# david-m-rosen/Optimization

Hardware: AMD Instinct MI355X
Metric: TNT Steihaug-CG HVP+inner-product throughput (higher is better)
Workload: dtype f64

## Files before the change

### optimization_amd/csrc/context.hip

```cpp
#include "mi_internal.h"
#include <chrono>
#include <cstring>
#include <strings.h>
#include <unistd.h>

#include <dlfcn.h>

namespace mi {

static thread_local char g_err[1024] = "";

void set_error(const char *fmt, ...) {
  va_list ap;
  va_start(ap, fmt);
  vsnprintf(g_err, sizeof(g_err), fmt, ap);
  va_end(ap);
}

int hip_fail(hipError_t e, const char *what, const char *file, int line) {
  set_error("HIP error %d (%s) in %s at %s:%d", (int)e, hipGetErrorString(e), what, file, line);
  (void)hipGetLastError();
  if (e == hipErrorNoDevice || e == hipErrorInvalidDevice) return MI_ERR_NO_DEVICE;
  if (e == hipErrorOutOfMemory) return MI_ERR_OOM;
  return MI_ERR_HIP;
// ... 171 lines not shown
using namespace mi;

namespace {
struct OptionDesc {
  const char *name;
  int (*set)(mi_ctx *, long);
  bool integer = false;
};
#define OPT_BOOL(FN, FIELD) \
  int FN(mi_ctx *c, long v) { c->FIELD = v != 0; return MI_OK; }
OPT_BOOL(opt_force_slot_path, force_slot_path)
OPT_BOOL(opt_force_lockstep, force_lockstep)
OPT_BOOL(opt_no_dirgram, no_dirgram)
OPT_BOOL(opt_dirgram_direct, dirgram_direct)
OPT_BOOL(opt_force_uniform_grid, cfg.force_uniform_grid)
OPT_BOOL(opt_no_fold, cfg.no_fold)
OPT_BOOL(opt_halo_push_late, cfg.halo_push_late)
OPT_BOOL(opt_no_packed, cfg.no_packed)
OPT_BOOL(opt_no_window, cfg.no_window)
OPT_BOOL(opt_no_win_bounds, cfg.no_win_bounds)
OPT_BOOL(opt_no_far_computed, cfg.no_far_computed)
OPT_BOOL(opt_words16, cfg.words16)
OPT_BOOL(opt_no_spmm_stream, cfg.no_spmm_stream)
OPT_BOOL(opt_no_spmm_win, cfg.no_spmm_win)
OPT_BOOL(opt_no_spmm_sweep, cfg.no_spmm_sweep)
OPT_BOOL(opt_no_zero_copy, cfg.no_zero_copy)
OPT_BOOL(opt_no_polled_sync, cfg.no_polled_sync)
OPT_BOOL(opt_no_update_mfma, cfg.no_update_mfma)
OPT_BOOL(opt_halo_rprime, cfg.halo_rprime)
OPT_BOOL(opt_no_gram_half, cfg.no_gram_half)
OPT_BOOL(opt_so3_no_quat, cfg.so3_no_quat)
OPT_BOOL(opt_so3_no_rquat, cfg.so3_no_rquat)
OPT_BOOL(opt_early_s, cfg.early_s)
OPT_BOOL(opt_no_update_pair, cfg.no_update_pair)
OPT_BOOL(opt_two_kernel_step, cfg.two_kernel_step)
OPT_BOOL(opt_warn_generic, warn_generic)
#undef OPT_BOOL
int opt_max_grid(mi_ctx *c, long v) {
  c->max_grid = (int)std::min<long>(kMaxGrid, std::max<long>(1, v));
  return MI_OK;
}
int opt_wide_quad(mi_ctx *c, long v) {
  c->cfg.wide_quad = v < 0 ? -1 : v != 0;
  return MI_OK;
}
int opt_wide_window(mi_ctx *c, long v) {
  c->cfg.wide_window = v < 0 ? -1 : v != 0;
  return MI_OK;
}
int opt_so3_sort_nbr(mi_ctx *c, long v) {
  c->cfg.so3_sort_nbr = (int)v;
  return MI_OK;
}
int opt_sweep_zsegs(mi_ctx *c, long v) {
  c->cfg.sweep_zsegs = (int)std::max<long>(0, std::min<long>(v, 1024));
  return MI_OK;
}
int opt_reanchor(mi_ctx *c, long v) {
  c->cfg.reanchor = (int)std::max<long>(0, std::min<long>(v, 1 << 20));
  return MI_OK;
}
int opt_ipc_timeout_ms(mi_ctx *c, long v) {
  c->cfg.ipc_timeout_ms = std::max<long>(0, v);
  return MI_OK;
}
const OptionDesc kOptions[] = {
    {"FORCE_SLOT_PATH", opt_force_slot_path}, {"FORCE_LOCKSTEP", opt_force_lockstep},
    {"NO_DIRGRAM", opt_no_dirgram}, {"DIRGRAM_DIRECT", opt_dirgram_direct}, {"MAX_GRID", opt_max_grid, true},
    {"FORCE_UNIFORM_GRID", opt_force_uniform_grid}, {"IPC_TIMEOUT_MS", opt_ipc_timeout_ms, true},
    {"NO_FOLD", opt_no_fold}, {"HALO_PUSH_LATE", opt_halo_push_late}, {"NO_PACKED", opt_no_packed},
    {"NO_WINDOW", opt_no_window}, {"NO_WIN_BOUNDS", opt_no_win_bounds}, {"NO_FAR_COMPUTED", opt_no_far_computed},
    {"WORDS16", opt_words16}, {"NO_SPMM_STREAM", opt_no_spmm_stream}, {"NO_SPMM_WIN", opt_no_spmm_win},
    {"NO_SPMM_SWEEP", opt_no_spmm_sweep}, {"SWEEP_ZSEGS", opt_sweep_zsegs, true},
    {"NO_ZERO_COPY", opt_no_zero_copy}, {"NO_POLLED_SYNC", opt_no_polled_sync}, {"WIDE_QUAD", opt_wide_quad, true}, {"WIDE_WINDOW", opt_wide_window, true},
    {"NO_UPDATE_MFMA", opt_no_update_mfma}, {"HALO_RPRIME", opt_halo_rprime}, {"NO_GRAM_HALF", opt_no_gram_half}, {"SO3_NO_QUAT", opt_so3_no_quat}, {"SO3_NO_RQUAT", opt_so3_no_rquat}, {"EARLY_S", opt_early_s}, {"NO_UPDATE_PAIR", opt_no_update_pair}, {"TWO_KERNEL_STEP", opt_two_kernel_step}, {"SO3_SORT_NBR", opt_so3_sort_nbr, true},
    {"WARN_GENERIC", opt_warn_generic}, {"REANCHOR", opt_reanchor, true},
};
bool option_value(const OptionDesc &o, const char *e, long *v) {
  char *end = nullptr;
  *v = strtol(e, &end, 0);
  if (end != e && *end == '\0') return true;
  if (o.integer) {
    fprintf(stderr, "[mi355opt] warning: MI355OPT_%s=\"%s\" is not an integer; ignored (the default stays)\n", o.name, e);
    return false;
  }
  *v = (!strcasecmp(e, "no") || !strcasecmp(e, "false") || !strcasecmp(e, "off")) ? 0 : 1;
  return true;
}
void config_from_env(mi_ctx *ctx) {
  for (const OptionDesc &o : kOptions) {
    char name[64];
    snprintf(name, sizeof(name), "MI355OPT_%s", o.name);
    long v = 0;
    if (const char *e = getenv(name))
      if (option_value(o, e, &v)) (void)o.set(ctx, v);
  }
  static bool warned = false;
  if (warned || !environ) return;
  warned = true;
  for (char **ep = environ; *ep; ++ep) {
    if (strncmp(*ep, "MI355OPT_", 9) != 0) continue;
    const char *nm = *ep + 9, *eq = strchr(nm, '=');
    const size_t len = eq ? (size_t)(eq - nm) : strlen(nm);
    bool known = false;
    for (const OptionDesc &o : kOptions) known |= strlen(o.name) == len && strncmp(o.name, nm, len) == 0;
    for (const char *h : {"LIB", "COMM", "BUILD_TAG", "EXTRA_CFLAGS", "NO_UNITY"})
      known |= strlen(h) == len && strncmp(h, nm, len) == 0;
    known |= len >= 6 && strncmp(nm, "BENCH_", 6) == 0;
// ... 297 lines not shown
```

### optimization_amd/csrc/mi_internal.h

```cpp
#pragma once

#include <hip/hip_runtime.h>

#include <cstdarg>
#include <cstdint>
#include <cstdio>
#include <cstring>
#include <map>
#include <string>
#include <set>
#include <vector>

#include "mi355opt.h"

namespace mi {

constexpr int kWave = 64;
constexpr int kBlock = 1024;
constexpr int kWaves = kBlock / kWave;
constexpr int kMaxP = 8;
constexpr int kMaxGrid = 512;
constexpr int kMaxRows = 1024;
constexpr int kMaxComps = 64;
constexpr int kNumXCD = 8;
// ... 8 lines not shown
    if (_e != hipSuccess) return ::mi::hip_fail(_e, #expr, __FILE__, __LINE__); \
  } while (0)

#define MI_TRY(expr)          \
  do {                        \
    int _s = (expr);          \
    if (_s != MI_OK) return _s; \
  } while (0)

#define MI_REQUIRE(cond, ...)              \
  do {                                     \
    if (!(cond)) {                         \
      ::mi::set_error(__VA_ARGS__);        \
      return MI_ERR_INVALID_ARGUMENT;      \
    }                                      \
  } while (0)

struct HostStatus {
  volatile uint64_t word;
  volatile uint32_t epoch;
};

struct CgState {
  double sk_M_pk, sk_M_2, pk_M_2;
  double target_rk_norm;
  double rv;
  double alpha, beta, kappa, sigma;
  double skplus1_M_2;
  double M_norm;
  unsigned long long k;
  unsigned long long launches;
  int mode;
  int exit_reason;
};
static_assert(sizeof(CgState) <= 128, "the CG state is meant to fit one 128-byte line");
struct CgConst {
  double Delta, Delta_2, epsilon;
  unsigned long long max_iterations;
  unsigned long long rag0, rag_per;
};
enum CgMode { CG_RUN = 0, CG_KERNEL_PENDING = 1, CG_APPLY_SIGMA = 2, CG_DONE = 3 };

struct Config {
  bool force_uniform_grid = false;
  long ipc_timeout_ms = 0;
  bool no_fold = false;
  bool halo_push_late = false;
  bool no_packed = false;
  bool no_window = false;
  bool no_win_bounds = false;
  bool no_far_computed = false;
  bool words16 = false;
  bool no_spmm_stream = false;
  bool no_spmm_sweep = true;
  int sweep_zsegs = 0;
  bool no_spmm_win = false;
  bool no_zero_copy = false;
  int wide_quad = -1;
  int wide_window = -1;
  bool no_polled_sync = false;
  bool two_kernel_step = false;
  int reanchor = 25;
  bool no_update_pair = false;
  bool no_gram_half = false;
  bool no_update_mfma = false;
  bool halo_rprime = false;
  bool early_s = false;
  bool so3_no_rquat = false;
  bool so3_no_quat = false;
  int so3_sort_nbr = 0;
};

struct KTimer {
  bool enabled = false;
  std::vector<std::pair<hipEvent_t, hipEvent_t>> pending;
  size_t launches = 0;
  double total_ms = 0;
};

}

struct mi_ctx {
  int device = -1;
  hipStream_t stream = nullptr;
  char device_name[128] = {0};
  int num_cu = 256;
  bool uniform_grid = false;
  int max_grid = 512;
  std::multimap<size_t, void *> pool_free;
  std::map<void *, size_t> pool_all;
  size_t pool_bytes = 0;
  void *control_slab = nullptr;
  double *partials = nullptr;
  double *partials_b = nullptr;
  double *partials2 = nullptr;
  double *partials_user = nullptr;
  double *scalars = nullptr;
  double *host_scalars = nullptr;
  mi::CgState *cg = nullptr;
  mi::CgState *cg1 = nullptr;
// ... 366 lines not shown
```

### optimization_amd/csrc/stpcg.hip

```cpp
#include "comm_ipc.h"
#include "mi_internal.h"
#include "stiefel_core.h"

#include <cmath>
#include <type_traits>

using namespace mi;

namespace {

enum { PRE_NONE = 0, PRE_DIAG = 1, PRE_BLOCK3 = 2, PRE_EXTERNAL = 3 };

__device__ __forceinline__ void publish(HostStatus *hs, unsigned long long launches, int done) {
  __hip_atomic_store(&hs->word, (uint64_t)(launches << 1) | (uint64_t)(done ? 1 : 0), __ATOMIC_RELAXED,
                     __HIP_MEMORY_SCOPE_SYSTEM);
}

#define CG_FIELDS(X)                                                                               \
  X(sk_M_pk) X(sk_M_2) X(pk_M_2) X(target_rk_norm) X(rv) X(alpha) X(beta)                          \
  X(kappa) X(sigma) X(skplus1_M_2) X(M_norm) X(k) X(launches) X(mode) X(exit_reason)
__device__ __forceinline__ CgState load_state(const CgState *__restrict__ src) {
  CgState s;
#define X(f) s.f = src->f;
  CG_FIELDS(X)
// ... 258 lines not shown
    s.exit_reason = MI_STPCG_EXIT_RESIDUAL;
    s.M_norm = sqrt(0.0);
  }
  store_state(st, s);
  publish(hs, 0, s.mode == CG_DONE);
}

struct DirGramArgs {
  const double *X, *Y, *S;
  double *gpartials;
  double *gdir;
  int ns;
};

#ifdef MI_FOLD_STAMPS
}
extern "C" __attribute__((visibility("default"))) int mi_debug_fold_stamp_buffer(void *dev_ptr) {
  return (int)hipMemcpyToSymbol(HIP_SYMBOL(mi::g_fold_stamps), &dev_ptr, sizeof(dev_ptr));
}
namespace {
#endif

template <int SP>
struct DirGramLds {
  static constexpr int value = (SymIdx<SP>::NS * kWaves > kWaves + 1) ? SymIdx<SP>::NS * kWaves : kWaves + 1;
};
template <>
struct DirGramLds<0> {
  static constexpr int value = kWaves + 1;
};
static_assert(kWaves + 1 >= kIpcVals, "LDS of the folded exchange");

#define CG_KERNEL_ATTR
#define CG_UPDATE_NAME k_cg_update
#define CG_PUPDATE_NAME k_cg_pupdate
#include "stpcg_kernels.inc"
#undef CG_KERNEL_ATTR
#undef CG_UPDATE_NAME
#undef CG_PUPDATE_NAME
#define CG_KERNEL_ATTR __attribute__((amdgpu_num_sgpr(80), amdgpu_waves_per_eu(8, 8)))
#define CG_UPDATE_NAME k_cg_update_s80
#define CG_PUPDATE_NAME k_cg_pupdate_s80
#include "stpcg_kernels.inc"
#undef CG_KERNEL_ATTR
#undef CG_UPDATE_NAME
#undef CG_PUPDATE_NAME

template <class F>
__device__ __forceinline__ void reduce_rows_1x512(const double *__restrict__ partials, int count, double &out, double *lds,
                                                  F &&after_issue) {
  const int lane = threadIdx.x & 63, w = threadIdx.x >> 6;
  double t[8];
#pragma unroll
  for (int j = 0; j < 8; ++j) t[j] = 0.0;
  if (w == 0) {
#pragma unroll
    for (int j = 0; j < 8; ++j) {
      const int r = lane + 64 * j;
      if (r < count) t[j] = partials[r];
    }
  }
  after_issue();
  if (w == 0) {
    double v = 0;
#pragma unroll
    for (int j = 0; j < 8; ++j) v += t[j];
    v = wave_reduce_sum(v);
    if (lane == 0) lds[0] = v;
  }
  __syncthreads();
  out = lds[0];
  __syncthreads();
}

__global__ __launch_bounds__(kBlock) __attribute__((amdgpu_waves_per_eu(8, 8))) void k_cg_pupdate_early(
    size_t n, CgConst cc, const CgState *__restrict__ st_in, CgState *__restrict__ st_out,
    const double *__restrict__ partials_b, int nparts_b, const double *__restrict__ v, double *__restrict__ p,
    double *__restrict__ s, HostStatus *hs, double *__restrict__ trace, size_t trace_cap, DirGramArgs dg) {
  __shared__ double lds[kWaves + 1];
// ... 57 lines not shown
      trace[3 * trace_cap + k] = cs.rv;
    }
    publish(hs, cs.launches, cs.mode == CG_DONE);
    if (dg.gdir && mode_in == CG_RUN && cs.mode == CG_RUN) {
      for (int i = 0; i < dg.ns; ++i) dg.gdir[SLOT_GDIR_P + i] = -dg.gdir[i] + cs.beta * dg.gdir[SLOT_GDIR_P + i];
    }
  }
  if (mode_in == CG_KERNEL_PENDING) {
    const double sigma = cs.sigma;
    for (unsigned i = i0; i < n2; i += stride) {
      const double2 pv = reinterpret_cast<const double2 *>(p)[i];
      double2 sv = reinterpret_cast<double2 *>(s)[i];
      sv.x += sigma * pv.x; sv.y += sigma * pv.y;
      reinterpret_cast<double2 *>(s)[i] = sv;
    }
    if ((n & 1) && leader) s[n - 1] += sigma * p[n - 1];
  } else if (mode_in == CG_RUN) {
    const double alpha = cs.alpha, beta = cs.beta;
    const bool dir = cs.mode == CG_RUN;
    if (dir) {
#pragma unroll
      for (int j = 0; j < 3; ++j)
        if (Le[j] < n2) {
          double2 pv = pe[j];
          const double2 vv = ve[j];
          pv.x = -vv.x + beta * pv.x; pv.y = -vv.y + beta * pv.y;
          reinterpret_cast<double2 *>(p)[Le[j]] = pv;
        }
    }
    if ((n & 1) && leader) {
      s[n - 1] = s[n - 1] + alpha * p[n - 1];
      if (dir) p[n - 1] = -v[n - 1] + beta * p[n - 1];
    }
  }
}


template <int NS>
__global__ __launch_bounds__(kBlock) void k_cg_step2(size_t n, CgConst cc, const CgState *__restrict__ st_in,
                                                     CgState *__restrict__ st_out, const double *__restrict__ partials_a,
                                                     int nparts_a, const double *__restrict__ Hp, double *__restrict__ r,
                                                     double *__restrict__ p, double *__restrict__ s, HostStatus *hs,
                                                     double *__restrict__ trace, size_t trace_cap, DirGramArgs dg) {
  constexpr int KC = 3 + NS + 2;
  __shared__ double lds[3 * (kWaves + 1)];
  static_assert(KC <= kWaves, "one wave per component");
  CgState cs = load_state(st_in);
  const bool leader = blockIdx.x == 0 && threadIdx.x == 0;
  if (cs.mode == CG_DONE) {
    if (leader) store_state(st_out, cs);
    return;
  }
  const size_t n2 = n >> 1, stride = (size_t)gridDim.x * kBlock, i0 = (size_t)blockIdx.x * kBlock + threadIdx.x;
  double2 hv0 = make_double2(0, 0), rv0 = hv0, pv0 = hv0, sv0 = hv0;
  auto prefetch = [&] {
    if (i0 < n2) {
      hv0 = reinterpret_cast<const double2 *>(Hp)[i0];
      rv0 = reinterpret_cast<double2 *>(r)[i0];
      pv0 = reinterpret_cast<double2 *>(p)[i0];
      sv0 = reinterpret_cast<double2 *>(s)[i0];
    }
  };
  double d[KC];
  reduce_rows<KC>(partials_a, nparts_a, d, lds, prefetch);
  step_a(cs, cc, d[0], d[1], d[2]);
  const int mode_a = cs.mode;
// ... 316 lines not shown
  touch(s_out);
  ctx->fusion.fused_stpcg_solves++;
  MI_REQUIRE(!P || (P->ctx == ctx && P->n == g->n), "preconditioner dimension/context mismatch");
  MI_REQUIRE(!prm->constraint_At || (P && P->apply_project),
             "constraint_At needs a constraint preconditioner (mi_precon_create_constraint)");
  MI_REQUIRE(!(P && P->kind == 3 && ctx->world_size > 1),
             "the constraint preconditioner is single-rank: its reductions are not completed across ranks");
  MI_REQUIRE(prm->Delta > 0, "Trust-region radius (Delta) must be a positive real value");
  MI_REQUIRE(prm->kappa_fgr >= 0 && prm->kappa_fgr < 1,
             "Target fractional reduction of the gradient norm (kappa_fgr) must be a real value in "
             "the range [0,1)");
  MI_REQUIRE(prm->theta >= 0 && prm->theta <= 1,
             "Target superlinear convergence rate (theta) must be a real value in the range [0,1]");
  MI_REQUIRE(prm->epsilon > 0 && prm->epsilon < 1,
             "Relative norm tolerance for declaring a vector to lie in the kernel of H (epsilon) "
             "should be a small positive number in the range (0,1)");

  RangeScope range("mi_stpcg");
  comm_halo_fold_drop(ctx);
  const size_t n = g->n;
  const int pre = !P ? PRE_NONE : (P->kind == 1 ? PRE_DIAG : (P->kind == 2 ? PRE_BLOCK3 : PRE_EXTERNAL));
  MI_REQUIRE(pre != PRE_BLOCK3 || n % 3 == 0, "block-Jacobi preconditioner needs n divisible by 3");
  const bool sharded = slot_mode(ctx);
  const bool rows = rows_mode(ctx);
  const mi_dirgram *dgp = (!ctx->no_dirgram && H->dirgram && H->apply_dir) ? H->dirgram : nullptr;
  if (dgp && dgp->p > 4 && (pre != PRE_NONE || ctx->dirgram_direct)) dgp = nullptr;
  MI_REQUIRE(!dgp || (dgp->p >= 1 && dgp->p <= kMaxP && dgp->n * (size_t)dgp->p == g->n),
             "operator's direction-Gram description does not match the problem dimension");
  const int run_ahead = prm->run_ahead > 0 ? prm->run_ahead : 3;
  const bool lockstep = (ctx->comm != nullptr && ctx->world_size > 1) || ctx->force_lockstep;

  if (P && P->fail_word) MI_HIP(hipMemsetAsync(P->fail_word, 0, sizeof(double), ctx->stream));

  mi_vec *r = nullptr, *v = nullptr, *p = nullptr, *Hp = nullptr;
  MI_TRY(mi_vec_create(ctx, n, &r));
  MI_TRY(mi_vec_create(ctx, n, &p));
  MI_TRY(mi_vec_create(ctx, n, &Hp));
  if (pre != PRE_NONE) MI_TRY(mi_vec_create(ctx, n, &v));
  double *vd = (pre == PRE_NONE) ? r->d : v->d;
  const double *pred = P ? P->data : nullptr;

  size_t tcap = 0;
  if (trace && trace->cap) {
    if (ctx->trace_cap < trace->cap) {
      if (ctx->trace_dev) MI_HIP(hipFree(ctx->trace_dev));
      MI_HIP(hipMalloc((void **)&ctx->trace_dev, 4 * trace->cap * sizeof(double)));
      ctx->trace_cap = trace->cap;
    }
    tcap = ctx->trace_cap;
  }

  ctx->cg_deferred = false;
  ctx->cg_deferred_seq = 0;
  ctx->epoch++;
  ctx->status->word = 0;
  ctx->status->epoch = ctx->epoch;

  CgSetup cfg{prm->Delta, prm->kappa_fgr, prm->theta, prm->epsilon,
              (unsigned long long)prm->max_iterations};
  CgConst cc{prm->Delta, prm->Delta * prm->Delta, prm->epsilon, (unsigned long long)prm->max_iterations, 0ull, 0ull};
  hipStream_t st = ctx->stream;
  const int grid = (pre == PRE_BLOCK3) ? grid_for(ctx, n / 3, 2) : grid_for(ctx, n, 4);
  {
    const size_t n2 = n >> 1, step = (size_t)grid * kBlock;
    cc.rag0 = (n2 / step) * step;
    cc.rag_per = (n2 - cc.rag0 + (size_t)grid - 1) / (size_t)grid;
  }
  const bool recur = dgp && pre == PRE_NONE && !ctx->dirgram_direct;
  const int gns = dgp ? dgp->p * (dgp->p + 1) / 2 : 0;
  const DirGramArgs dga = dgp ? DirGramArgs{dgp->X, dgp->Y, dgp->S, ctx->partials2,
                                            recur ? ctx->scalars + SLOT_GDIR : nullptr, gns}
                              : DirGramArgs{nullptr, nullptr, nullptr, nullptr, nullptr, 0};
  const int sp = (dgp && !recur) ? dgp->p : 0;
  const int kc = recur ? dir_comps(dgp->p) : 3;
  double *slots_g = ctx->scalars + SLOT_GRAM;
  double *slots_a = ctx->scalars + SLOT_CG, *slots_b = ctx->scalars + SLOT_CG + 4;
  CgState *st0 = ctx->cg, *st1 = ctx->cg1;
  const bool folded = sharded && recur && kc <= kIpcVals && comm_fold_enabled(ctx) && !ctx->force_slot_path;
  bool rprime = false;
  if (recur && !folded && dgp->halo_A) {
    const int st_rp = comm_rprime_prepare(ctx, dgp->halo_A, &rprime);
    if (st_rp != MI_OK) {
      mi_vec_destroy(r);
      mi_vec_destroy(p);
      mi_vec_destroy(Hp);
      if (v) mi_vec_destroy(v);
      return st_rp;
    }
  }
  const bool init_fused = recur && n == dgp->n * (size_t)dgp->p;
  const bool gdir_in_scalar_init = recur && !sharded && !rows;
  const bool twok = ctx->cfg.two_kernel_step && recur && dgp->twok && dgp->p == 3 && !sharded && !rows && !lockstep &&
                    init_fused && gdir_in_scalar_init;
  CgState *st_final = st0;
  double *tr = tcap ? ctx->trace_dev : nullptr;
  int ret = MI_OK;
  ctx->cg_live = st0;

#define CG_CHECK(expr)   \
  do {                   \
    int _s = (expr);     \
    if (_s != MI_OK) {   \
      ret = _s;          \
      goto cleanup;      \
    }                    \
  } while (0)
#define LAUNCH_PRE(KERNEL, ...)                                                                   \
  switch (pre) {                                                                                  \
    case PRE_NONE: hipLaunchKernelGGL((KERNEL<PRE_NONE>), dim3(grid), dim3(kBlock), 0, st, __VA_ARGS__); break;     \
    case PRE_DIAG: hipLaunchKernelGGL((KERNEL<PRE_DIAG>), dim3(grid), dim3(kBlock), 0, st, __VA_ARGS__); break;     \
    case PRE_BLOCK3: hipLaunchKernelGGL((KERNEL<PRE_BLOCK3>), dim3(grid), dim3(kBlock), 0, st, __VA_ARGS__); break; \
    default: hipLaunchKernelGGL((KERNEL<PRE_EXTERNAL>), dim3(grid), dim3(kBlock), 0, st, __VA_ARGS__); break;       \
  }
#define LAUNCH_UPDATE(FS)                                                                              \
  switch (pre) {                                                                                       \
    case PRE_NONE: hipLaunchKernelGGL((k_cg_update<PRE_NONE, FS>), dim3(grid), dim3(kBlock), 0, st, UPD_ARGS, NoFold{}); break;     \
    case PRE_DIAG: hipLaunchKernelGGL((k_cg_update<PRE_DIAG, FS>), dim3(grid), dim3(kBlock), 0, st, UPD_ARGS, NoFold{}); break;     \
    case PRE_BLOCK3: hipLaunchKernelGGL((k_cg_update<PRE_BLOCK3, FS>), dim3(grid), dim3(kBlock), 0, st, UPD_ARGS, NoFold{}); break; \
    default: hipLaunchKernelGGL((k_cg_update<PRE_EXTERNAL, FS>), dim3(grid), dim3(kBlock), 0, st, UPD_ARGS, NoFold{}); break;       \
  }

  if (init_fused) {
    KScope ks(ctx, MI_K_CG_INIT);
    const size_t nrows = dgp->n;
#define INIT_DG(SPV)                                                                                       \
  hipLaunchKernelGGL(k_cg_init_dirgram<SPV>, dim3(grid), dim3(StBlk<SPV>::threads), 0, st, nrows, (const double *)g->d, \
                     r->d, p->d, s_out->d, ctx->partials_b, dga)
    switch (dgp->p) {
      case 1: INIT_DG(1); break;
      case 2: INIT_DG(2); break;
      case 3: INIT_DG(3); break;
      case 4: INIT_DG(4); break;
      case 5: INIT_DG(5); break;
      case 6: INIT_DG(6); break;
      case 7: INIT_DG(7); break;
      default: INIT_DG(8); break;
    }
#undef INIT_DG
  } else {
    KScope ks(ctx, MI_K_CG_INIT);
    LAUNCH_PRE(k_cg_init, n, (const double *)g->d, pred, r->d, vd, p->d, s_out->d, ctx->partials_b);
  }
  if (pre == PRE_EXTERNAL) {
    if (P->apply_project) CG_CHECK(P->apply_project(P, r, v, prm->constraint_At));
    else CG_CHECK(P->apply(P, r, v));
    hipLaunchKernelGGL(k_cg_dot_rv<true>, dim3(grid), dim3(kBlock), 0, st, n, (const CgState *)st0,
                       (const double *)r->d, (const double *)v->d, p->d, ctx->partials_b);
  }
  if (dgp) {
    const size_t nrows = dgp->n;
    if (!init_fused) {
      switch (dgp->p) {
// ... 70 lines not shown
            hipLaunchKernelGGL(k_cg_gdir_anchor, dim3(1), dim3(kBlock), 0, st, (const double *)ctx->partials2, grid, gns,
                               (const double *)slots_g, sharded ? 1 : 0, (const CgState *)st0,
                               dga.gdir + (which == 0 ? SLOT_GDIR_P : 0), (double *)nullptr);
          }
        }
      }

      int nparts = 0;
      if (twok) {
        CgState *cur = (k & 1) ? st1 : st0, *nxt = (k & 1) ? st0 : st1;
        ctx->cg_live = cur;
        ctx->twok_r = r->d;
        CG_CHECK(H->apply_dir(H, p, Hp, -2, &nparts));
        ctx->twok_r = nullptr;
        ++hvp;
        {
          KScope ks(ctx, MI_K_CG_UPDATE);
          hipLaunchKernelGGL(k_cg_step2<6>, dim3(grid), dim3(kBlock), 0, st, n, cc, (const CgState *)cur, nxt,
                             (const double *)ctx->partials, nparts, (const double *)Hp->d, r->d, p->d, s_out->d,
                             ctx->status_dev, tr, tcap, dga);
        }
        st_final = nxt;
        continue;
      }
      if (dgp) {
        CG_CHECK(H->apply_dir(H, p, Hp, recur ? -1 : grid, &nparts));
      } else if (H->apply_dots) {
        CG_CHECK(H->apply_dots(H, p, Hp, &nparts));
      } else {
        CG_CHECK(H->apply(H, p, Hp));
        CG_CHECK(launch_dot3_partials(ctx, n, p->d, Hp->d, &nparts));
      }
      ++hvp;
#define UPD_ARGS                                                                                      \
  n, cc, (const CgState *)st0, st1, (const double *)ctx->partials, nparts,                              \
      (const double *)(recur ? slots_g : slots_a), (const double *)p->d, (const double *)Hp->d, pred,  \
      s_out->d, r->d, vd, ctx->partials_b, dga
      if (recur) {
#define UPD_RECUR(KN, FS, FT, FV)                                                                                  \
  switch (kc) {                                                                                                    \
    case 4: hipLaunchKernelGGL((KN<PRE_NONE, FS, 4, FT>), dim3(grid), dim3(kBlock), 0, st, UPD_ARGS, FV); break;   \
    case 6: hipLaunchKernelGGL((KN<PRE_NONE, FS, 6, FT>), dim3(grid), dim3(kBlock), 0, st, UPD_ARGS, FV); break;   \
    case 9: hipLaunchKernelGGL((KN<PRE_NONE, FS, 9, FT>), dim3(grid), dim3(kBlock), 0, st, UPD_ARGS, FV); break;   \
    default: hipLaunchKernelGGL((k_cg_update_s80<PRE_NONE, FS, 16, FT>), dim3(grid), dim3(kBlock), 0, st, UPD_ARGS, FV); break; \
  }
#define UPD_WIDE(FS)                                                                                                        \
  switch (kc) {                                                                                                             \
    case 18: hipLaunchKernelGGL((k_cg_update<PRE_NONE, FS, 18, NoFold>), dim3(grid), dim3(kBlock), 0, st, UPD_ARGS, NoFold{}); break; \
    case 24: hipLaunchKernelGGL((k_cg_update<PRE_NONE, FS, 24, NoFold>), dim3(grid), dim3(kBlock), 0, st, UPD_ARGS, NoFold{}); break; \
    case 31: hipLaunchKernelGGL((k_cg_update<PRE_NONE, FS, 31, NoFold>), dim3(grid), dim3(kBlock), 0, st, UPD_ARGS, NoFold{}); break; \
    default: hipLaunchKernelGGL((k_cg_update<PRE_NONE, FS, 39, NoFold>), dim3(grid), dim3(kBlock), 0, st, UPD_ARGS, NoFold{}); break; \
  }
        if (kc > 16) {
          if (sharded) CG_CHECK(reduce_rows_allreduce(ctx, ctx->partials, nparts, kc, slots_g));
          else if (rows) CG_CHECK(comm_allreduce_rows(ctx, ctx->partials, kc));
          KScope ks(ctx, MI_K_CG_UPDATE);
          if (sharded) { UPD_WIDE(true); } else { UPD_WIDE(false); }
        } else if (sharded && folded) {
          const FoldArgs fold_a = comm_fold_next(ctx);
          KScope ks(ctx, MI_K_CG_UPDATE);
          UPD_RECUR(k_cg_update_s80, false, FoldArgs, fold_a);
        } else if (sharded) {
          CG_CHECK(reduce_rows_allreduce(ctx, ctx->partials, nparts, kc, slots_g));
          KScope ks(ctx, MI_K_CG_UPDATE);
          UPD_RECUR(k_cg_update_s80, true, NoFold, NoFold{});
        } else {
          if (rows) CG_CHECK(comm_allreduce_rows(ctx, ctx->partials, kc));
          KScope ks(ctx, MI_K_CG_UPDATE);
          UPD_RECUR(k_cg_update, false, NoFold, NoFold{});
        }
#undef UPD_RECUR
#undef UPD_WIDE
      } else if (sharded) {
        CG_CHECK(reduce_rows_allreduce(ctx, ctx->partials, nparts, 3, slots_a));
        KScope ks(ctx, MI_K_CG_UPDATE);
        LAUNCH_UPDATE(true);
      } else {
        if (rows) CG_CHECK(comm_allreduce_rows(ctx, ctx->partials, 3));
        KScope ks(ctx, MI_K_CG_UPDATE);
        LAUNCH_UPDATE(false);
      }
#undef UPD_ARGS
      if (pre == PRE_EXTERNAL) {
        if (P->apply_project) CG_CHECK(P->apply_project(P, r, v, prm->constraint_At));
        else CG_CHECK(P->apply(P, r, v));
        hipLaunchKernelGGL(k_cg_dot_rv<false>, dim3(grid), dim3(kBlock), 0, st, n, (const CgState *)st1,
                           (const double *)r->d, (const double *)v->d, p->d, ctx->partials_b);
      }
#define PUPD_ARGS                                                                                          \
  n, cc, (const CgState *)st1, st0, (const double *)ctx->partials_b, grid, (const double *)slots_b,        \
      (const double *)vd, p->d, s_out->d, ctx->status_dev, tr, tcap, dga
#define PUPD(KN, FS, SPV) \
  hipLaunchKernelGGL((KN<FS, SPV>), dim3(grid), dim3(kBlock), 0, st, PUPD_ARGS, NoFold{})
#define LAUNCH_PUPD(KN0, KN1, FS)               \
  switch (sp) {                                 \
    case 0: PUPD(KN0, FS, 0); break;            \
    case 1: PUPD(KN1, FS, 1); break;            \
    case 2: PUPD(k_cg_pupdate, FS, 2); break;   \
    case 3: PUPD(k_cg_pupdate, FS, 3); break;   \
    default: PUPD(k_cg_pupdate, FS, 4); break;  \
  }
      if (sharded && folded) {
        const FoldArgs fold_b = comm_fold_next(ctx);
        FoldPush fp{fold_b, HaloPush{}};
        const bool push = dgp && dgp->halo_A && k + 1 < prm->max_iterations &&
                          comm_halo_fold_next(ctx, dgp->halo_A, dgp->p, p->d, &fp.h);
        KScope ks(ctx, MI_K_CG_PUPDATE);
        if (push)
          hipLaunchKernelGGL((k_cg_pupdate_s80<false, 0, FoldPush>), dim3(grid), dim3(kBlock), 0, st, PUPD_ARGS, fp);
        else
          hipLaunchKernelGGL((k_cg_pupdate_s80<false, 0, FoldArgs>), dim3(grid), dim3(kBlock), 0, st, PUPD_ARGS, fold_b);
      } else if (sharded) {
        CG_CHECK(reduce_rows_allreduce(ctx, ctx->partials_b, grid, 1, slots_b));
        if (rprime) CG_CHECK(comm_rprime_exchange(ctx, dgp->halo_A, dgp->p, r->d, nullptr, 0));
        KScope ks(ctx, MI_K_CG_PUPDATE);
        LAUNCH_PUPD(k_cg_pupdate_s80, k_cg_pupdate_s80, true);
      } else {
        if (rows && rprime) CG_CHECK(comm_rprime_exchange(ctx, dgp->halo_A, dgp->p, r->d, ctx->partials_b, 1));
        else if (rows) CG_CHECK(comm_allreduce_rows(ctx, ctx->partials_b, 1));
        KScope ks(ctx, MI_K_CG_PUPDATE);
        const bool early = sp == 0 && !rows && ctx->cfg.early_s && grid <= 512 && cc.rag0 <= 2ull * (size_t)grid * kBlock &&
                           (n >> 1) < ((size_t)1 << 31);
        if (early)
          hipLaunchKernelGGL(k_cg_pupdate_early, dim3(grid), dim3(kBlock), 0, st, n, cc, (const CgState *)st1, st0,
                             (const double *)ctx->partials_b, grid, (const double *)vd, p->d, s_out->d, ctx->status_dev, tr,
                             tcap, dga);
        else
          LAUNCH_PUPD(k_cg_pupdate, k_cg_pupdate_s80, false);
      }
      if (rprime && (sharded || rows)) {
        const double *hr = nullptr;
        double *hp = nullptr;
        size_t cnt = 0;
        comm_rprime_buffers(ctx, dgp->halo_A, dgp->p, &hr, &hp, &cnt);
        if (cnt) {
          const int hg = (int)std::max<size_t>(1, std::min<size_t>((cnt + 255) / 256, 512));
          hipLaunchKernelGGL(k_halo_dir, dim3(hg), dim3(256), 0, st, (const CgState *)st0, hr, hp, cnt);
        }
        comm_rprime_mark(ctx, dgp->halo_A, dgp->p, p->d);
      }
#undef LAUNCH_PUPD
#undef PUPD
#undef PUPD_ARGS
    }
    result->hvp_calls = hvp;
    comm_halo_fold_drop(ctx);
  }

  if (prm->defer_result && !(trace && trace->cap)) {
    hipError_t e = hipSuccess;
    *precon_fail_host(ctx) = 0.0;
    ctx->cg_deferred_seq = result_to_host(ctx, st_final, P);
    if (!ctx->cg_deferred_seq) {
      if (!ctx->cg_deferred_ev) e = hipEventCreateWithFlags(&ctx->cg_deferred_ev, hipEventDisableTiming);
      if (e == hipSuccess) e = hipMemcpyAsync(ctx->cg_host, st_final, sizeof(CgState), hipMemcpyDeviceToHost, st);
      if (e == hipSuccess && P && P->fail_word)
        e = hipMemcpyAsync(precon_fail_host(ctx), P->fail_word, sizeof(double), hipMemcpyDeviceToHost, st);
      if (e == hipSuccess) e = hipEventRecord(ctx->cg_deferred_ev, st);
    }
    if (e != hipSuccess) CG_CHECK(hip_fail(e, "stpcg deferred read-back", __FILE__, __LINE__));
    ctx->cg_deferred = true;
// ... 23 lines not shown
      if (ipc_err) {
        set_error("a wait in the peer-memory exchange layer timed out: the result of this solve is invalid");
        ret = MI_ERR_COMM;
        goto cleanup;
      }
    }
    const CgState &f = *ctx->cg_host;
    result->update_step_M_norm = f.M_norm;
    result->num_iterations = (size_t)f.k;
    result->exit_reason = f.exit_reason;
    result->rv_final = f.rv;
    if (trace && trace->cap) {
      const size_t len = f.k < trace->cap ? (size_t)f.k : trace->cap;
      trace->len = len;
      double *dst[4] = {trace->alpha, trace->beta, trace->kappa, trace->rv};
      for (int c = 0; c < 4; ++c)
        if (dst[c] && len) {
          e = hipMemcpy(dst[c], ctx->trace_dev + (size_t)c * tcap, len * sizeof(double),
                        hipMemcpyDeviceToHost);
          if (e != hipSuccess) CG_CHECK(hip_fail(e, "stpcg trace copy", __FILE__, __LINE__));
        }
    }
  }

cleanup:
#undef CG_CHECK
#undef LAUNCH_PRE
#undef LAUNCH_UPDATE
  ctx->cg_live = nullptr;
  comm_halo_fold_drop(ctx);
  if (ret != MI_OK) (void)hipStreamSynchronize(st);
  mi_vec_destroy(r);
  mi_vec_destroy(p);
  mi_vec_destroy(Hp);
  mi_vec_destroy(v);
  return ret;
}

}
```

### optimization_amd/csrc/stpcg_kernels.inc

```

template <int PRE, bool FROM_SLOTS, int KC = 3, class FOLD = NoFold>
__global__ __launch_bounds__(kBlock) CG_KERNEL_ATTR void CG_UPDATE_NAME(size_t n, CgConst cc, const CgState *__restrict__ st_in,
                                                      CgState *__restrict__ st_out,
                                                      const double *__restrict__ partials_a, int nparts_a,
                                                      const double *__restrict__ slots,
                                                      const double *__restrict__ p,
                                                      const double *__restrict__ Hp,
                                                      const double *__restrict__ pre,
                                                      double *__restrict__ s, double *__restrict__ r,
                                                      double *__restrict__ v,
                                                      double *__restrict__ partials_b, DirGramArgs dg,
                                                      FOLD fold) {
  __shared__ double lds[3 * (kWaves + 1)];
  static_assert(KC >= 3 && KC <= 3 * (kWaves + 1), "3 curvature dots + at most 36 Gram components (p <= 8)");
  CgState cs = load_state(st_in);
  if (cs.mode == CG_DONE) {
    if (blockIdx.x == 0 && threadIdx.x == 0) store_state(st_out, cs);
    return;
  }
  FOLD_STAMP(0);
  const size_t n2 = n >> 1, stride = (size_t)gridDim.x * kBlock;
  const size_t i0 = (size_t)blockIdx.x * kBlock + threadIdx.x;
  auto next_of = [&](size_t i_) -> size_t { return i_ + stride; };
  const size_t ifirst = i0;
// ... 4 lines not shown
      hv0 = reinterpret_cast<const double2 *>(Hp)[ifirst];
      rv0 = reinterpret_cast<double2 *>(r)[ifirst];
    }
  };
  auto prefetch = [&] {
    if (kFolded && threadIdx.x < 64) return;
    prefetch_now();
  };
  double d[KC];
  if (FROM_SLOTS) {
    prefetch_now();
#pragma unroll
    for (int i = 0; i < KC; ++i) d[i] = slots[i];
  } else {
    reduce_rows<KC>(partials_a, nparts_a, d, lds, prefetch);
    fold_maybe<KC>(d, fold, lds);
    if (kFolded && threadIdx.x < 64) prefetch_now();
    if (!kFolded) FOLD_STAMP(1);
  }
  step_a(cs, cc, d[0], d[1], d[2]);
  if (!kFolded) FOLD_STAMP(5);
  if (blockIdx.x == 0 && threadIdx.x == 0) {
    store_state(st_out, cs);
    if (KC > 3 && cs.mode == CG_RUN) {
#pragma unroll
      for (int i = 0; i < KC - 3; ++i)
        if (i < dg.ns) dg.gdir[i] = dg.gdir[i] + cs.alpha * d[3 + i];
    }
  }

  const int mode = cs.mode;
  double acc[1] = {0};
  if (mode == CG_APPLY_SIGMA) {
    const double sigma = cs.sigma;
    for (size_t i = i0; i < n2; i += stride) {
      const double2 pv = reinterpret_cast<const double2 *>(p)[i];
      double2 sv = reinterpret_cast<double2 *>(s)[i];
      sv.x += sigma * pv.x; sv.y += sigma * pv.y;
      reinterpret_cast<double2 *>(s)[i] = sv;
    }
    if ((n & 1) && blockIdx.x == 0 && threadIdx.x == 0) s[n - 1] += sigma * p[n - 1];
    return;
  }
  if (mode == CG_KERNEL_PENDING) {
    for (size_t i = i0; i < n2; i += stride) {
      const double2 pv = reinterpret_cast<const double2 *>(p)[i];
      const double2 rv = reinterpret_cast<const double2 *>(r)[i];
      acc[0] += pv.x * rv.x; acc[0] += pv.y * rv.y;
    }
    if ((n & 1) && blockIdx.x == 0 && threadIdx.x == 0) acc[0] += p[n - 1] * r[n - 1];
  } else {
    const double alpha = cs.alpha;
    if (PRE == PRE_BLOCK3) {
      const size_t nb = n / 3;
      for (size_t b = i0; b < nb; b += stride) {
        double rr[3];
#pragma unroll
        for (int c = 0; c < 3; ++c) {
          const size_t i = 3 * b + c;
          rr[c] = r[i] + alpha * Hp[i];
          r[i] = rr[c];
        }
        const double *M = pre + 9 * b;
#pragma unroll
        for (int c = 0; c < 3; ++c) {
          const double vv = M[3 * c] * rr[0] + M[3 * c + 1] * rr[1] + M[3 * c + 2] * rr[2];
// ... 208 lines not shown
```

Before: 5701.

## Defer the s-vector update to every other CG iteration using a double-buffered direction

Adds a default-on DEFER_S path. The s += alpha*p update is skipped on even iterations, and the old direction is kept in a second buffer p2 so the odd-iteration p-update kernel can apply both alpha_prev*p_old and alpha*p_new to s in one pass. The aim is to halve the read-modify-write traffic on s. The cost is an extra n-length vector, a new pupdate kernel, an extra CgState field, and more loads in the flush iteration. Correctness at termination and in the sigma boundary cases depends on the flush logic handling those paths.

```diff
diff --git a/optimization_amd/csrc/context.hip b/optimization_amd/csrc/context.hip
--- a/optimization_amd/csrc/context.hip
+++ b/optimization_amd/csrc/context.hip
@@ -227,6 +227,7 @@
 OPT_BOOL(opt_so3_no_quat, cfg.so3_no_quat)
 OPT_BOOL(opt_so3_no_rquat, cfg.so3_no_rquat)
 OPT_BOOL(opt_early_s, cfg.early_s)
+OPT_BOOL(opt_defer_s, cfg.defer_s)
 OPT_BOOL(opt_no_update_pair, cfg.no_update_pair)
 OPT_BOOL(opt_two_kernel_step, cfg.two_kernel_step)
 OPT_BOOL(opt_warn_generic, warn_generic)
@@ -268,7 +269,7 @@
     {"WORDS16", opt_words16}, {"NO_SPMM_STREAM", opt_no_spmm_stream}, {"NO_SPMM_WIN", opt_no_spmm_win},
     {"NO_SPMM_SWEEP", opt_no_spmm_sweep}, {"SWEEP_ZSEGS", opt_sweep_zsegs, true},
     {"NO_ZERO_COPY", opt_no_zero_copy}, {"NO_POLLED_SYNC", opt_no_polled_sync}, {"WIDE_QUAD", opt_wide_quad, true}, {"WIDE_WINDOW", opt_wide_window, true},
-    {"NO_UPDATE_MFMA", opt_no_update_mfma}, {"HALO_RPRIME", opt_halo_rprime}, {"NO_GRAM_HALF", opt_no_gram_half}, {"SO3_NO_QUAT", opt_so3_no_quat}, {"SO3_NO_RQUAT", opt_so3_no_rquat}, {"EARLY_S", opt_early_s}, {"NO_UPDATE_PAIR", opt_no_update_pair}, {"TWO_KERNEL_STEP", opt_two_kernel_step}, {"SO3_SORT_NBR", opt_so3_sort_nbr, true},
+    {"NO_UPDATE_MFMA", opt_no_update_mfma}, {"HALO_RPRIME", opt_halo_rprime}, {"NO_GRAM_HALF", opt_no_gram_half}, {"SO3_NO_QUAT", opt_so3_no_quat}, {"SO3_NO_RQUAT", opt_so3_no_rquat}, {"EARLY_S", opt_early_s}, {"DEFER_S", opt_defer_s}, {"NO_UPDATE_PAIR", opt_no_update_pair}, {"TWO_KERNEL_STEP", opt_two_kernel_step}, {"SO3_SORT_NBR", opt_so3_sort_nbr, true},
     {"WARN_GENERIC", opt_warn_generic}, {"REANCHOR", opt_reanchor, true},
 };
 bool option_value(const OptionDesc &o, const char *e, long *v) {
diff --git a/optimization_amd/csrc/mi_internal.h b/optimization_amd/csrc/mi_internal.h
--- a/optimization_amd/csrc/mi_internal.h
+++ b/optimization_amd/csrc/mi_internal.h
@@ -64,6 +64,7 @@
   unsigned long long launches;
   int mode;
   int exit_reason;
+  double alpha_prev;
 };
 static_assert(sizeof(CgState) <= 128, "the CG state is meant to fit one 128-byte line");
 struct CgConst {
@@ -98,6 +99,7 @@
   bool no_update_mfma = false;
   bool halo_rprime = false;
   bool early_s = false;
+  bool defer_s = true;
   bool so3_no_rquat = false;
   bool so3_no_quat = false;
   int so3_sort_nbr = 0;
diff --git a/optimization_amd/csrc/stpcg.hip b/optimization_amd/csrc/stpcg.hip
--- a/optimization_amd/csrc/stpcg.hip
+++ b/optimization_amd/csrc/stpcg.hip
@@ -314,6 +314,7 @@
 static_assert(kWaves + 1 >= kIpcVals, "LDS of the folded exchange");
 
 #define CG_KERNEL_ATTR
+#define CG_UPDATE_SIGMA 1
 #define CG_UPDATE_NAME k_cg_update
 #define CG_PUPDATE_NAME k_cg_pupdate
 #include "stpcg_kernels.inc"
@@ -327,6 +328,23 @@
 #undef CG_KERNEL_ATTR
 #undef CG_UPDATE_NAME
 #undef CG_PUPDATE_NAME
+#undef CG_UPDATE_SIGMA
+#define CG_UPDATE_SIGMA 0
+#define CG_KERNEL_ATTR
+#define CG_UPDATE_NAME k_cg_update_ns
+#define CG_PUPDATE_NAME k_cg_pupdate_ns_unused
+#include "stpcg_kernels.inc"
+#undef CG_KERNEL_ATTR
+#undef CG_UPDATE_NAME
+#undef CG_PUPDATE_NAME
+#define CG_KERNEL_ATTR __attribute__((amdgpu_num_sgpr(80), amdgpu_waves_per_eu(8, 8)))
+#define CG_UPDATE_NAME k_cg_update_ns_s80
+#define CG_PUPDATE_NAME k_cg_pupdate_ns_s80_unused
+#include "stpcg_kernels.inc"
+#undef CG_KERNEL_ATTR
+#undef CG_UPDATE_NAME
+#undef CG_PUPDATE_NAME
+#undef CG_UPDATE_SIGMA
 
 template <class F>
 __device__ __forceinline__ void reduce_rows_1x512(const double *__restrict__ partials, int count, double &out, double *lds,
@@ -450,6 +468,115 @@
       s[n - 1] = s[n - 1] + alpha * p[n - 1];
       if (dir) p[n - 1] = -v[n - 1] + beta * p[n - 1];
     }
+  }
+}
+
+
+template <bool FLUSH>
+__global__ __launch_bounds__(kBlock) __attribute__((amdgpu_waves_per_eu(8, 8))) void k_cg_pupdate_ds(
+    size_t n, CgConst cc, const CgState *__restrict__ st_in, CgState *__restrict__ st_out,
+    const double *__restrict__ partials_b, int nparts_b, const double *__restrict__ v, const double *__restrict__ pc,
+    double *__restrict__ px, double *__restrict__ s, HostStatus *hs, double *__restrict__ trace, size_t trace_cap,
+    DirGramArgs dg) {
+  __shared__ double lds[kWaves + 1];
+  CgState cs = load_state(st_in);
+  const bool leader = blockIdx.x == 0 && threadIdx.x == 0;
+  if (cs.mode == CG_DONE) {
+    if (leader) store_state(st_out, cs);
+    return;
+  }
+  const int mode_in = cs.mode;
+  const size_t n2 = n >> 1, stride = (size_t)gridDim.x * kBlock;
+  const size_t i0 = (size_t)blockIdx.x * kBlock + threadIdx.x;
+  const size_t tail0 = cc.rag0, per = cc.rag_per;
+  const size_t irem = (threadIdx.x < per) ? tail0 + (size_t)blockIdx.x * per + threadIdx.x : n2;
+  auto next_of = [&](size_t i_) -> size_t {
+    const size_t j_ = i_ + stride;
+    return j_ < tail0 ? j_ : ((i_ < tail0 && irem < n2) ? irem : n2);
+  };
+  const size_t ifirst = i0 < tail0 ? i0 : (irem < n2 ? irem : n2);
+  double2 vv0 = make_double2(0, 0), pv0 = vv0, ov0 = vv0, sv0 = vv0;
+  auto prefetch_now = [&] {
+    if (ifirst < n2) {
+      vv0 = reinterpret_cast<const double2 *>(v)[ifirst];
+      pv0 = reinterpret_cast<const double2 *>(pc)[ifirst];
+      if (FLUSH) {
+        ov0 = reinterpret_cast<double2 *>(px)[ifirst];
+        sv0 = reinterpret_cast<double2 *>(s)[ifirst];
+      }
+    }
+  };
+  double red[1] = {0};
+  if (mode_in != CG_APPLY_SIGMA) reduce_rows<1>(partials_b, nparts_b, red, lds, prefetch_now);
+  else prefetch_now();
+  step_b(cs, cc, red[0]);
+  cs.launches = cs.launches + 1;
+  const bool dir = mode_in == CG_RUN && cs.mode == CG_RUN;
+  if (leader) {
+    store_state(st_out, cs);
+    if (!FLUSH && dir) st_out->alpha_prev = cs.alpha;
+    if (mode_in == CG_RUN && trace && cs.k - 1 < trace_cap) {
+      const size_t k = (size_t)(cs.k - 1);
+      trace[k] = cs.alpha;
+      trace[trace_cap + k] = cs.beta;
+      trace[2 * trace_cap + k] = cs.kappa;
+      trace[3 * trace_cap + k] = cs.rv;
+    }
+    publish(hs, cs.launches, cs.mode == CG_DONE);
+    if (dg.gdir && dir) {
+      for (int i = 0; i < dg.ns; ++i) dg.gdir[SLOT_GDIR_P + i] = -dg.gdir[i] + cs.beta * dg.gdir[SLOT_GDIR_P + i];
+    }
+  }
+  const double beta = cs.beta;
+  if (FLUSH) {
+    const double alpha_old = st_out->alpha_prev, alpha = mode_in == CG_RUN ? cs.alpha : cs.sigma;
+    double2 vv = vv0, pv = pv0, ov = ov0, sv = sv0;
+    for (size_t i = ifirst; i < n2;) {
+      const size_t inext = next_of(i);
+      double2 vn = vv, pn = pv, on = ov, sn = sv;
+      if (inext < n2) {
+        vn = reinterpret_cast<const double2 *>(v)[inext];
+        pn = reinterpret_cast<const double2 *>(pc)[inext];
+        on = reinterpret_cast<double2 *>(px)[inext];
+        sn = reinterpret_cast<double2 *>(s)[inext];
+      }
+      sv.x = sv.x + alpha_old * ov.x; sv.y = sv.y + alpha_old * ov.y;
+      sv.x = sv.x + alpha * pv.x; sv.y = sv.y + alpha * pv.y;
+      reinterpret_cast<double2 *>(s)[i] = sv;
+      if (dir) {
+        pv.x = -vv.x + beta * pv.x; pv.y = -vv.y + beta * pv.y;
+        reinterpret_cast<double2 *>(px)[i] = pv;
+      }
+      i = inext; vv = vn; pv = pn; ov = on; sv = sn;
+    }
+    if ((n & 1) && leader) {
+      s[n - 1] = s[n - 1] + alpha_old * px[n - 1];
+      s[n - 1] = s[n - 1] + alpha * pc[n - 1];
+      if (dir) px[n - 1] = -v[n - 1] + beta * pc[n - 1];
+    }
+  } else if (dir) {
+    double2 vv = vv0, pv = pv0;
+    for (size_t i = ifirst; i < n2;) {
+      const size_t inext = next_of(i);
+      double2 vn = vv, pn = pv;
+      if (inext < n2) {
+        vn = reinterpret_cast<const double2 *>(v)[inext];
+        pn = reinterpret_cast<const double2 *>(pc)[inext];
+      }
+      pv.x = -vv.x + beta * pv.x; pv.y = -vv.y + beta * pv.y;
+      reinterpret_cast<double2 *>(px)[i] = pv;
+      i = inext; vv = vn; pv = pn;
+    }
+    if ((n & 1) && leader) px[n - 1] = -v[n - 1] + beta * pc[n - 1];
+  } else if (mode_in != CG_APPLY_SIGMA) {
+    const double alpha = mode_in == CG_RUN ? cs.alpha : cs.sigma;
+    for (size_t i = i0; i < n2; i += stride) {
+      const double2 pv = reinterpret_cast<const double2 *>(pc)[i];
+      double2 sv = reinterpret_cast<double2 *>(s)[i];
+      sv.x = sv.x + alpha * pv.x; sv.y = sv.y + alpha * pv.y;
+      reinterpret_cast<double2 *>(s)[i] = sv;
+    }
+    if ((n & 1) && leader) s[n - 1] = s[n - 1] + alpha * pc[n - 1];
   }
 }
 
@@ -832,7 +959,7 @@
 
   if (P && P->fail_word) MI_HIP(hipMemsetAsync(P->fail_word, 0, sizeof(double), ctx->stream));
 
-  mi_vec *r = nullptr, *v = nullptr, *p = nullptr, *Hp = nullptr;
+  mi_vec *r = nullptr, *v = nullptr, *p = nullptr, *p2 = nullptr, *Hp = nullptr;
   MI_TRY(mi_vec_create(ctx, n, &r));
   MI_TRY(mi_vec_create(ctx, n, &p));
   MI_TRY(mi_vec_create(ctx, n, &Hp));
@@ -892,9 +1019,22 @@
   const bool gdir_in_scalar_init = recur && !sharded && !rows;
   const bool twok = ctx->cfg.two_kernel_step && recur && dgp->twok && dgp->p == 3 && !sharded && !rows && !lockstep &&
                     init_fused && gdir_in_scalar_init;
+  const bool early = !sharded && !rows && sp == 0 && ctx->cfg.early_s && grid <= 512 &&
+                     cc.rag0 <= 2ull * (size_t)grid * kBlock && (n >> 1) < ((size_t)1 << 31);
+  const bool defer = !sharded && !rows && !lockstep && !twok && sp == 0 && !early && ctx->cfg.defer_s;
   CgState *st_final = st0;
   double *tr = tcap ? ctx->trace_dev : nullptr;
   int ret = MI_OK;
+  if (defer) {
+    const int st_p2 = mi_vec_create(ctx, n, &p2);
+    if (st_p2 != MI_OK) {
+      mi_vec_destroy(r);
+      mi_vec_destroy(p);
+      mi_vec_destroy(Hp);
+      if (v) mi_vec_destroy(v);
+      return st_p2;
+    }
+  }
   ctx->cg_live = st0;
 
 #define CG_CHECK(expr)   \
@@ -912,12 +1052,12 @@
     case PRE_BLOCK3: hipLaunchKernelGGL((KERNEL<PRE_BLOCK3>), dim3(grid), dim3(kBlock), 0, st, __VA_ARGS__); break; \
     default: hipLaunchKernelGGL((KERNEL<PRE_EXTERNAL>), dim3(grid), dim3(kBlock), 0, st, __VA_ARGS__); break;       \
   }
-#define LAUNCH_UPDATE(FS)                                                                              \
+#define LAUNCH_UPDATE(KN, FS)                                                                          \
   switch (pre) {                                                                                       \
-    case PRE_NONE: hipLaunchKernelGGL((k_cg_update<PRE_NONE, FS>), dim3(grid), dim3(kBlock), 0, st, UPD_ARGS, NoFold{}); break;     \
-    case PRE_DIAG: hipLaunchKernelGGL((k_cg_update<PRE_DIAG, FS>), dim3(grid), dim3(kBlock), 0, st, UPD_ARGS, NoFold{}); break;     \
-    case PRE_BLOCK3: hipLaunchKernelGGL((k_cg_update<PRE_BLOCK3, FS>), dim3(grid), dim3(kBlock), 0, st, UPD_ARGS, NoFold{}); break; \
-    default: hipLaunchKernelGGL((k_cg_update<PRE_EXTERNAL, FS>), dim3(grid), dim3(kBlock), 0, st, UPD_ARGS, NoFold{}); break;       \
+    case PRE_NONE: hipLaunchKernelGGL((KN<PRE_NONE, FS>), dim3(grid), dim3(kBlock), 0, st, UPD_ARGS, NoFold{}); break;     \
+    case PRE_DIAG: hipLaunchKernelGGL((KN<PRE_DIAG, FS>), dim3(grid), dim3(kBlock), 0, st, UPD_ARGS, NoFold{}); break;     \
+    case PRE_BLOCK3: hipLaunchKernelGGL((KN<PRE_BLOCK3, FS>), dim3(grid), dim3(kBlock), 0, st, UPD_ARGS, NoFold{}); break; \
+    default: hipLaunchKernelGGL((KN<PRE_EXTERNAL, FS>), dim3(grid), dim3(kBlock), 0, st, UPD_ARGS, NoFold{}); break;       \
   }
 
   if (init_fused) {
@@ -1054,53 +1194,55 @@
         CG_CHECK(launch_dot3_partials(ctx, n, p->d, Hp->d, &nparts));
       }
       ++hvp;
+      const bool sigma_later = defer && (k & 1);
 #define UPD_ARGS                                                                                      \
   n, cc, (const CgState *)st0, st1, (const double *)ctx->partials, nparts,                              \
       (const double *)(recur ? slots_g : slots_a), (const double *)p->d, (const double *)Hp->d, pred,  \
       s_out->d, r->d, vd, ctx->partials_b, dga
       if (recur) {
-#define UPD_RECUR(KN, FS, FT, FV)                                                                                  \
+#define UPD_RECUR(KN, K16, FS, FT, FV)                                                                             \
   switch (kc) {                                                                                                    \
     case 4: hipLaunchKernelGGL((KN<PRE_NONE, FS, 4, FT>), dim3(grid), dim3(kBlock), 0, st, UPD_ARGS, FV); break;   \
     case 6: hipLaunchKernelGGL((KN<PRE_NONE, FS, 6, FT>), dim3(grid), dim3(kBlock), 0, st, UPD_ARGS, FV); break;   \
     case 9: hipLaunchKernelGGL((KN<PRE_NONE, FS, 9, FT>), dim3(grid), dim3(kBlock), 0, st, UPD_ARGS, FV); break;   \
-    default: hipLaunchKernelGGL((k_cg_update_s80<PRE_NONE, FS, 16, FT>), dim3(grid), dim3(kBlock), 0, st, UPD_ARGS, FV); break; \
-  }
-#define UPD_WIDE(FS)                                                                                                        \
+    default: hipLaunchKernelGGL((K16<PRE_NONE, FS, 16, FT>), dim3(grid), dim3(kBlock), 0, st, UPD_ARGS, FV); break; \
+  }
+#define UPD_WIDE(KN, FS)                                                                                                    \
   switch (kc) {                                                                                                             \
-    case 18: hipLaunchKernelGGL((k_cg_update<PRE_NONE, FS, 18, NoFold>), dim3(grid), dim3(kBlock), 0, st, UPD_ARGS, NoFold{}); break; \
-    case 24: hipLaunchKernelGGL((k_cg_update<PRE_NONE, FS, 24, NoFold>), dim3(grid), dim3(kBlock), 0, st, UPD_ARGS, NoFold{}); break; \
-    case 31: hipLaunchKernelGGL((k_cg_update<PRE_NONE, FS, 31, NoFold>), dim3(grid), dim3(kBlock), 0, st, UPD_ARGS, NoFold{}); break; \
-    default: hipLaunchKernelGGL((k_cg_update<PRE_NONE, FS, 39, NoFold>), dim3(grid), dim3(kBlock), 0, st, UPD_ARGS, NoFold{}); break; \
+    case 18: hipLaunchKernelGGL((KN<PRE_NONE, FS, 18, NoFold>), dim3(grid), dim3(kBlock), 0, st, UPD_ARGS, NoFold{}); break; \
+    case 24: hipLaunchKernelGGL((KN<PRE_NONE, FS, 24, NoFold>), dim3(grid), dim3(kBlock), 0, st, UPD_ARGS, NoFold{}); break; \
+    case 31: hipLaunchKernelGGL((KN<PRE_NONE, FS, 31, NoFold>), dim3(grid), dim3(kBlock), 0, st, UPD_ARGS, NoFold{}); break; \
+    default: hipLaunchKernelGGL((KN<PRE_NONE, FS, 39, NoFold>), dim3(grid), dim3(kBlock), 0, st, UPD_ARGS, NoFold{}); break; \
   }
         if (kc > 16) {
           if (sharded) CG_CHECK(reduce_rows_allreduce(ctx, ctx->partials, nparts, kc, slots_g));
           else if (rows) CG_CHECK(comm_allreduce_rows(ctx, ctx->partials, kc));
           KScope ks(ctx, MI_K_CG_UPDATE);
-          if (sharded) { UPD_WIDE(true); } else { UPD_WIDE(false); }
+          if (sharded) { UPD_WIDE(k_cg_update, true); } else if (sigma_later) { UPD_WIDE(k_cg_update_ns, false); } else { UPD_WIDE(k_cg_update, false); }
         } else if (sharded && folded) {
           const FoldArgs fold_a = comm_fold_next(ctx);
           KScope ks(ctx, MI_K_CG_UPDATE);
-          UPD_RECUR(k_cg_update_s80, false, FoldArgs, fold_a);
+          UPD_RECUR(k_cg_update_s80, k_cg_update_s80, false, FoldArgs, fold_a);
         } else if (sharded) {
           CG_CHECK(reduce_rows_allreduce(ctx, ctx->partials, nparts, kc, slots_g));
           KScope ks(ctx, MI_K_CG_UPDATE);
-          UPD_RECUR(k_cg_update_s80, true, NoFold, NoFold{});
+          UPD_RECUR(k_cg_update_s80, k_cg_update_s80, true, NoFold, NoFold{});
         } else {
           if (rows) CG_CHECK(comm_allreduce_rows(ctx, ctx->partials, kc));
           KScope ks(ctx, MI_K_CG_UPDATE);
-          UPD_RECUR(k_cg_update, false, NoFold, NoFold{});
+          if (sigma_later) { UPD_RECUR(k_cg_update_ns, k_cg_update_ns_s80, false, NoFold, NoFold{}); }
+          else { UPD_RECUR(k_cg_update, k_cg_update_s80, false, NoFold, NoFold{}); }
         }
 #undef UPD_RECUR
 #undef UPD_WIDE
       } else if (sharded) {
         CG_CHECK(reduce_rows_allreduce(ctx, ctx->partials, nparts, 3, slots_a));
         KScope ks(ctx, MI_K_CG_UPDATE);
-        LAUNCH_UPDATE(true);
+        LAUNCH_UPDATE(k_cg_update, true);
       } else {
         if (rows) CG_CHECK(comm_allreduce_rows(ctx, ctx->partials, 3));
         KScope ks(ctx, MI_K_CG_UPDATE);
-        LAUNCH_UPDATE(false);
+        if (sigma_later) { LAUNCH_UPDATE(k_cg_update_ns, false); } else { LAUNCH_UPDATE(k_cg_update, false); }
       }
 #undef UPD_ARGS
       if (pre == PRE_EXTERNAL) {
@@ -1141,14 +1283,24 @@
         if (rows && rprime) CG_CHECK(comm_rprime_exchange(ctx, dgp->halo_A, dgp->p, r->d, ctx->partials_b, 1));
         else if (rows) CG_CHECK(comm_allreduce_rows(ctx, ctx->partials_b, 1));
         KScope ks(ctx, MI_K_CG_PUPDATE);
-        const bool early = sp == 0 && !rows && ctx->cfg.early_s && grid <= 512 && cc.rag0 <= 2ull * (size_t)grid * kBlock &&
-                           (n >> 1) < ((size_t)1 << 31);
-        if (early)
+#define PUPD_DS(FLUSH)                                                                                                  \
+  hipLaunchKernelGGL(k_cg_pupdate_ds<FLUSH>, dim3(grid), dim3(kBlock), 0, st, n, cc, (const CgState *)st1, st0,          \
+                     (const double *)ctx->partials_b, grid, (const double *)vd, (const double *)p->d, p2->d, s_out->d, \
+                     ctx->status_dev, tr, tcap, dga)
+        if (early) {
           hipLaunchKernelGGL(k_cg_pupdate_early, dim3(grid), dim3(kBlock), 0, st, n, cc, (const CgState *)st1, st0,
                              (const double *)ctx->partials_b, grid, (const double *)vd, p->d, s_out->d, ctx->status_dev, tr,
                              tcap, dga);
-        else
+        } else if (defer && (k & 1)) {
+          PUPD_DS(true);
+          std::swap(p, p2);
+        } else if (defer && k + 1 < prm->max_iterations) {
+          PUPD_DS(false);
+          std::swap(p, p2);
+        } else {
           LAUNCH_PUPD(k_cg_pupdate, k_cg_pupdate_s80, false);
+        }
+#undef PUPD_DS
       }
       if (rprime && (sharded || rows)) {
         const double *hr = nullptr;
@@ -1238,6 +1390,7 @@
   if (ret != MI_OK) (void)hipStreamSynchronize(st);
   mi_vec_destroy(r);
   mi_vec_destroy(p);
+  mi_vec_destroy(p2);
   mi_vec_destroy(Hp);
   mi_vec_destroy(v);
   return ret;
diff --git a/optimization_amd/csrc/stpcg_kernels.inc b/optimization_amd/csrc/stpcg_kernels.inc
--- a/optimization_amd/csrc/stpcg_kernels.inc
+++ b/optimization_amd/csrc/stpcg_kernels.inc
@@ -60,6 +60,7 @@
   const int mode = cs.mode;
   double acc[1] = {0};
   if (mode == CG_APPLY_SIGMA) {
+    if (!CG_UPDATE_SIGMA) return;
     const double sigma = cs.sigma;
     for (size_t i = i0; i < n2; i += stride) {
       const double2 pv = reinterpret_cast<const double2 *>(p)[i];
```

Measured after the change: 5850, median of 6. +2.6%, better.
